# yitian97/SDformerFlow

Measured on AMD Instinct MI355X. Metric: event-frames/sec fwd (1x10x2x288x384), higher is better.
Workload: dtype f16x2; 1 GPU; BASELINE configs[1]: MS_SpikingformerFlowNet_en4 forward, batch 1 per GPU, 10-bin 288x384 voxel, neuron=lif; a step = one forward of one sample; 2 HIP streams per GPU, each replaying the HIP graph of one launch sequence that carries 10 independent batch-1 forwards of different voxels (replicas: every flow map bit-equal to a separate batch-1 forward, asserted by --full runs); one process per GPU; in_flight=2, replicas_per_launch=10, samples_in_flight=20, hip_graph=True, weight_planes=2

## Files before the change

sdformerflow_amd/csrc/ms_smallm.hip:

```cpp
#include "wide_common.h"
#include "switches.h"
#include <stdlib.h>

#ifdef SDF_STAMP
__device__ unsigned long long g_smallm_stamp[4 * 8];
__device__ unsigned long long g_smallm_census[2 * 1024];
#define MSTAMP(i) do { st[i] = __builtin_readcyclecounter(); } while (0)
#else
#define MSTAMP(i)
#endif

namespace sdfmm {
namespace {

struct SmallMParams {
  const uint8_t* A;
  const int8_t* W;
  const float* cscale;
  int N, K, HW;
  int64_t P;
  const float *bias, *alpha, *beta;
  const float* resid;
  float* out;
  int ldo;
  uint8_t* out_spike;
  int ldsp;
  SdfNeuronCfg sn;
  float inv_tau;
  int ncg, nunits;
  int cv_H, cv_W, cv_Cin, cv_spt;
  int cv_inv;
};

template <int T, int EPI, int NK, int AM, bool BT, int CB>
__global__ __launch_bounds__(256, CB == 2 ? 2 : 1) void smallm_kernel(SmallMParams P) {
  constexpr int RB = RBW, NS = CB == 2 ? 1 : 2, NBUF = NS + 1, ROWS = 16 * RB, SLOTS = 4 * RB, PPG = SLOTS / T, PPW = 4 * PPG, BN = 16 * CB;
  constexpr int SP1 = s_pitch(16), REDC = 3 * 2 * RB * 64 * 16;
  constexpr int STRIPB = 4 * RB * 1024, REDB = CB * REDC;
  static_assert(SLOTS % T == 0, "T must divide the 20 accumulator slots of a lane");
  static_assert(ROWS * SP1 <= REDC && STRIPB <= REDB, "the byte tiles and the strips lie inside the reduction buffer");
  __shared__ __attribute__((aligned(16))) uint8_t smem[REDB];
  __shared__ int32_t rowtab[ROWS];
  __shared__ uint32_t masktab[AM == 1 ? ROWS : 1];
  __shared__ __attribute__((aligned(16))) float psn_tbl[NK == 1 ? PSN_TABLE(T) : 4];
  const int tid = threadIdx.x, lane = tid & 63, wave = __builtin_amdgcn_readfirstlane(tid >> 6);
  const int l16 = lane & 15, lq = lane >> 4;
  int item = blockIdx.x;
  const int G = gridDim.x;
  if ((G & 7) == 0) item = (item & 7) * (G >> 3) + (item >> 3);
  if (item >= P.ncg * P.nunits) return;
#ifdef SDF_STAMP
  unsigned long long st[8] = {0, 0, 0, 0, 0, 0, 0, 0};
  const unsigned long long rt0 = __builtin_amdgcn_s_memrealtime();
  auto stamp_out = [&]() __attribute__((always_inline)) {
    asm volatile("s_waitcnt vmcnt(0)" ::: "memory");
    MSTAMP(5);
    if (lane == 0 && wave == 0 && blockIdx.x < 1024) {
      g_smallm_census[2 * blockIdx.x] = rt0;
      g_smallm_census[2 * blockIdx.x + 1] = __builtin_amdgcn_s_memrealtime();
    }
    if (lane == 0 && blockIdx.x == gridDim.x / 2) {
      unsigned long long* o = g_smallm_stamp + 8 * wave;
      for (int i = 0; i < 5; ++i) o[i] = st[i + 1] > st[i] ? st[i + 1] - st[i] : 0;
      o[5] = st[5] - st[0]; o[6] = __builtin_amdgcn_s_memrealtime() - rt0; o[7] = gridDim.x;
    }
  };
#endif
  MSTAMP(0);
  const int cg = item / P.nunits, unit = item - cg * P.nunits;
  const int n0 = cg * BN, K = P.K, N = P.N, HW = P.HW;
  const __amdgpu_buffer_rsrc_t A_rs = make_rsrc(P.A), W_rs = make_rsrc(P.W);
  const int nst = K >> 6;

  uint32_t pf[6] = {0, 0, 0, 0, 0, 0};
  if constexpr (BT) {
    const int per = G >> 3, first = (blockIdx.x & 7) * per;
    const uint32_t nw = 4u * (uint32_t)per, wi = 4u * (uint32_t)((blockIdx.x >> 3)) + (uint32_t)wave;
    const int cg_lo = first / P.nunits, cg_hi = min(P.ncg - 1, (first + per - 1) / P.nunits);
    const uint32_t cgb = (uint32_t)(CB * nst) * 3072u, wbase = (uint32_t)cg_lo * cgb, wlines = ((uint32_t)(cg_hi - cg_lo + 1) * cgb) >> 7;
    const uint32_t Lw = (wlines + nw - 1) / nw;
#pragma unroll
    for (int j = 0; j < 4; ++j) {
      const uint32_t ln = 64u * j + lane, line = wi * Lw + ln;
      pf[j] = __builtin_amdgcn_raw_buffer_load_b32(W_rs, (ln < Lw && line < wlines) ? wbase + line * 128u : INV, 0, 0);
    }
    const uint32_t alines = (uint32_t)(((int64_t)P.P * T * (AM == 1 ? P.cv_Cin : K)) >> 7), La = (alines + nw - 1) / nw;
#pragma unroll
    for (int j = 0; j < 2; ++j) {
      const uint32_t ln = 64u * j + lane, line = wi * La + ln;
      pf[4 + j] = __builtin_amdgcn_raw_buffer_load_b32(A_rs, (ln < La && line < alines) ? line * 128u : INV, 0, 0);
    }
  }

  if (tid < ROWS) {
    const int rb = tid >> 4, i = tid & 15, qq = i >> 2, slot = 4 * rb + (i & 3);
    const int pp = slot / T, t = slot - pp * T;
    const uint32_t pos = (uint32_t)unit * PPW + qq * PPG + pp;
    int32_t g = -1;
    if (pos < (uint32_t)P.P) {
      const uint32_t b = pos / (uint32_t)HW, hw = pos - b * (uint32_t)HW;
      g = (int32_t)((b * T + t) * (uint32_t)HW + hw);
    }
    rowtab[tid] = g;
    if constexpr (AM == 1) {
      uint32_t m = 0;
      if (g >= 0) {
        const uint32_t pix = (uint32_t)g % (uint32_t)HW, y = pix / (uint32_t)P.cv_W, xx = pix - y * (uint32_t)P.cv_W;
#pragma unroll
        for (int tp = 0; tp < 9; ++tp) {
          const int yy = (int)y + tp / 3 - 1, xw = (int)xx + tp % 3 - 1;
          if (yy >= 0 && yy < P.cv_H && xw >= 0 && xw < P.cv_W) m |= 1u << tp;
        }
      }
      masktab[tid] = m;
    }
  }
  if constexpr (NK == 1) psn_stage<T>(psn_tbl, P.sn, tid, 256);
  __syncthreads();
  uint32_t a_base[RB], a_mask[RB], b_off[CB];
  const int lr = lane >> 2, lp = (lane & 3) ^ ((lr >> 2) & 2);
#pragma unroll
  for (int rb = 0; rb < RB; ++rb) {
    const int32_t g = rowtab[16 * rb + lr];
    a_base[rb] = INV;
    a_mask[rb] = 0;
    if (g >= 0) {
      if constexpr (AM == 1) {
        a_base[rb] = (uint32_t)g * (uint32_t)P.cv_Cin + 16u * lp;
        a_mask[rb] = masktab[16 * rb + lr];
      } else {
        a_base[rb] = (uint32_t)g * (uint32_t)K + 16u * lp;
      }
    }
  }
#pragma unroll
  for (int cb = 0; cb < CB; ++cb) {
    if constexpr (BT) b_off[cb] = n0 + 16 * cb < N ? (uint32_t)(((n0 >> 4) + cb) * nst) * 3072u + 16u * lane : INV;
    else b_off[cb] = n0 + 16 * cb + l16 < N ? (uint32_t)(n0 + 16 * cb + l16) * (uint32_t)K + 16u * lq : INV;
  }
  uint8_t* mystrip = smem + wave * (RB * 1024);
  const uint32_t rd_off = (uint32_t)((4 * l16 + (lq ^ ((l16 >> 2) & 2))) * 16), wr_off = 16u * lane;

  i32x4 acc[3][RB][CB];
#pragma unroll
  for (int dg = 0; dg < 3; ++dg)
#pragma unroll
    for (int rb = 0; rb < RB; ++rb)
#pragma unroll
      for (int cb = 0; cb < CB; ++cb) acc[dg][rb][cb] = i32x4{0, 0, 0, 0};

  constexpr bool DBL = CB == 3;
  i32x4 araw[NS][RB], a2[DBL ? 2 : 1][RB], b[NBUF][3][CB];
  int sa_next = wave, sb_next = wave;
  const uint32_t plane = (uint32_t)N * (uint32_t)K;
#ifdef SMX_NOA
  constexpr bool XA = false;
#else
  constexpr bool XA = true;
#endif
#ifdef SMX_NOB
  constexpr bool XB = false;
#else
  constexpr bool XB = true;
#endif
  auto issue_a1 = [&](int ra, int rb) __attribute__((always_inline)) {
    if constexpr (AM == 1) {
      const int tap = (int)(((uint32_t)sa_next * (uint32_t)P.cv_inv) >> 16), cstep = sa_next - tap * P.cv_spt;
      const uint32_t toff = (uint32_t)(((tap / 3 - 1) * P.cv_W + (tap % 3 - 1)) * P.cv_Cin), cin0 = (uint32_t)cstep * 64u;
      const uint32_t ok = (0u - ((a_mask[rb] >> tap) & 1u)) & (0u - (uint32_t)XA);
      araw[ra][rb] = __builtin_bit_cast(i32x4, __builtin_amdgcn_raw_buffer_load_b128(A_rs, ((a_base[rb] + toff) & ok) | (INV & ~ok), cin0, 0));
    } else {
      const bool in = XA && sa_next < nst;
      araw[ra][rb] = __builtin_bit_cast(i32x4, __builtin_amdgcn_raw_buffer_load_b128(A_rs, in ? a_base[rb] : INV, (uint32_t)sa_next * 64u, 0));
    }
  };
  auto issue_b1 = [&](int rbuf, int f) __attribute__((always_inline)) {
    const bool in = XB && sb_next < nst;
    const int dg = f / CB, cb = f - dg * CB;
    const uint32_t so = BT ? (uint32_t)(sb_next * 3 + dg) * 1024u : (uint32_t)dg * plane + (uint32_t)sb_next * 64u;
    b[rbuf][dg][cb] = __builtin_bit_cast(i32x4, __builtin_amdgcn_raw_buffer_load_b128(W_rs, in ? b_off[cb] : INV, so, 0));
  };
  auto strip_write1 = [&](int ra, int rb) __attribute__((always_inline)) {
    *reinterpret_cast<i32x4*>(mystrip + rb * 1024 + wr_off) = araw[ra][rb];
  };
  auto strip_read1 = [&](int set, int rb) __attribute__((always_inline)) {
    a2[set][rb] = *reinterpret_cast<const i32x4*>(mystrip + rb * 1024 + rd_off);
  };
  auto step = [&](int i) __attribute__((always_inline)) {
    const int cur = DBL ? (i & 1) : 0, nxt = DBL ? (cur ^ 1) : 0;
#pragma unroll
    for (int g = 0; g < 3 * CB; ++g) {
      const int dg = g / CB, cb = g - dg * CB;
#pragma unroll
      for (int rb = 0; rb < RB; ++rb) {
#ifndef SMX_NOMFMA
        mfma_i8(acc[dg][rb][cb], a2[cur][rb], b[i % NBUF][dg][cb]);
#else
        asm volatile("" :: "v"(a2[cur][rb]), "v"(b[i % NBUF][dg][cb]));
#endif
        if (g == 0) strip_write1((i + 1) % NS, rb);
        if (g == 1) issue_a1((i + 1) % NS, rb);
        if (g == 2 && DBL) strip_read1(nxt, rb);
        if (g >= 1 && rb == (g == 1 ? RB - 1 : 0)) issue_b1(i % NBUF, g - 1);
        __builtin_amdgcn_sched_barrier(0);
      }
    }
    sa_next += 4;
    issue_b1(i % NBUF, 3 * CB - 1);
    sb_next += 4;
    if (!DBL) {
#pragma unroll
      for (int rb = 0; rb < RB; ++rb) strip_read1(nxt, rb);
    }
    __builtin_amdgcn_sched_barrier(0);
  };
  MSTAMP(1);
#pragma unroll
  for (int j = 0; j < NS; ++j) {
#pragma unroll
    for (int rb = 0; rb < RB; ++rb) issue_a1(j, rb);
    sa_next += 4;
  }
#pragma unroll
  for (int j = 0; j < NBUF; ++j) {
#pragma unroll
    for (int f = 0; f < 3 * CB; ++f) issue_b1(j, f);
    sb_next += 4;
  }
  asm volatile("" :: "v"(pf[0]), "v"(pf[1]), "v"(pf[2]), "v"(pf[3]), "v"(pf[4]), "v"(pf[5]));
#pragma unroll
  for (int rb = 0; rb < RB; ++rb) strip_write1(0, rb);
#pragma unroll
  for (int rb = 0; rb < RB; ++rb) issue_a1(0, rb);
  sa_next += 4;
#pragma unroll
  for (int rb = 0; rb < RB; ++rb) strip_read1(0, rb);
  __builtin_amdgcn_sched_barrier(0);
  constexpr int U = DBL ? 6 : 2;
  static_assert(U % NS == 0 && U % NBUF == 0, "ring sizes divide the round");
  const int nrounds = ((nst + 3) / 4 + U - 1) / U;
#pragma unroll 1
  for (int r = 0; r < nrounds; ++r) {
#pragma unroll
    for (int j = 0; j < U; ++j) step(j);
  }
  mfma_drain(acc);

  MSTAMP(2);
  const int c = lane & 15, q = lane >> 4;
  const bool owner = wave < CB;
  const int mycb = owner ? wave : 0;
  uint32_t xo[SLOTS];
  float res[SLOTS];
  float al = 1.f, be = 0.f, bs = 0.f, cs = 0.f;
  const int ncol = n0 + 16 * mycb + c;
  if (owner) {
#pragma unroll
    for (int s = 0; s < SLOTS; ++s) {
      const int32_t g = rowtab[16 * (s >> 2) + 4 * q + (s & 3)];
      xo[s] = (g >= 0 && ncol < N) ? ((uint32_t)g * (uint32_t)P.ldo + (uint32_t)ncol) * 4u : INV;
    }
    const __amdgpu_buffer_rsrc_t r_rs = make_rsrc(P.resid);
#pragma unroll
    for (int s = 0; s < SLOTS; ++s) res[s] = __builtin_bit_cast(float, __builtin_amdgcn_raw_buffer_load_b32(r_rs, P.resid ? xo[s] : INV, 0, 0));
    const int nc = ncol < N ? ncol : 0;
    al = P.alpha ? P.alpha[nc] : 1.f;
    be = P.alpha ? P.beta[nc] : 0.f;
    bs = P.bias ? P.bias[nc] : 0.f;
    cs = P.cscale[nc];
  }
  i32x4* red = reinterpret_cast<i32x4*>(smem);
  __builtin_amdgcn_sched_barrier(0);
  __syncthreads();
  __builtin_amdgcn_sched_barrier(0);
#pragma unroll
  for (int cb = 0; cb < CB; ++cb)
    if (wave != cb) {
      const int j = wave < cb ? wave : wave - 1;
#pragma unroll
      for (int rb = 0; rb < RB; ++rb) {
        red[(((cb * 3 + j) * 2 + 0) * RB + rb) * 64 + lane] = acc_read(acc[1][rb][cb]) * 256 + acc_read(acc[0][rb][cb]);
        red[(((cb * 3 + j) * 2 + 1) * RB + rb) * 64 + lane] = acc_read(acc[2][rb][cb]);
        __builtin_amdgcn_sched_barrier(0);
      }
    }
  __syncthreads();
  MSTAMP(3);
#ifdef SDF_STAMP
  if (!owner) { st[4] = st[3]; stamp_out(); return; }
#else
  if (!owner) return;
#endif
  const __amdgpu_buffer_rsrc_t x_rs = make_rsrc(P.out), o_rs = make_rsrc(P.out_spike);
  float val[SLOTS];
#pragma unroll
  for (int rb = 0; rb < RB; ++rb) {
    i32x4 lo = i32x4{0, 0, 0, 0}, hi = i32x4{0, 0, 0, 0};
#pragma unroll
    for (int cb = 0; cb < CB; ++cb)
      if (wave == cb) { lo = acc_read(acc[1][rb][cb]) * 256 + acc_read(acc[0][rb][cb]); hi = acc_read(acc[2][rb][cb]); }
#pragma unroll
    for (int j = 0; j < 3; ++j) {
      lo += red[(((mycb * 3 + j) * 2 + 0) * RB + rb) * 64 + lane];
      hi += red[(((mycb * 3 + j) * 2 + 1) * RB + rb) * 64 + lane];
    }
#pragma unroll
    for (int e = 0; e < 4; ++e) {
      const int s = 4 * rb + e;
      float v = __builtin_fmaf((float)hi[e], 65536.f, (float)lo[e]) * cs;
      v = v + bs;
      v = __builtin_fmaf(v, al, be);
      v = v + res[s];
      val[s] = v;
      if constexpr ((EPI & 2) != 0) __builtin_amdgcn_raw_buffer_store_b32(__builtin_bit_cast(uint32_t, v), x_rs, xo[s], 0, 0);
    }
    __builtin_amdgcn_sched_barrier(0);
  }
  if constexpr ((EPI & 1) != 0) {
    uint8_t* S = smem + mycb * REDC;
    uint32_t sel1, sel2;
    quad_sel(lane, sel1, sel2);
    const int m4 = (c >> 2), ci = c & 3;
    uint32_t bits = 0;
#pragma unroll
    for (int pp = 0; pp < PPG; ++pp) {
      float xs[T], sp[T];
#pragma unroll
      for (int t = 0; t < T; ++t) xs[t] = val[pp * T + t];
      neuron_any<NK, T>(xs, sp, P.sn, P.inv_tau, psn_tbl);
#pragma unroll
      for (int t = 0; t < T; ++t) bits |= ((__float_as_uint(sp[t]) >> 29) & 1u) << (pp * T + t);
    }
#pragma unroll
    for (int rb = 0; rb < RB; ++rb) {
      const uint32_t w = quad_tr_bytes(spread4(bits >> (4 * rb)), sel1, sel2);
      *reinterpret_cast<uint32_t*>(S + (16 * rb + 4 * q + ci) * SP1 + 4 * m4) = w;
    }
#pragma unroll
    for (int it = 0; it < (ROWS + 63) / 64; ++it) {
      const int r = lane + 64 * it;
      if (r < ROWS) {
        const int32_t g = rowtab[r];
        const u32x4 v = *reinterpret_cast<const u32x4*>(S + r * SP1);
        const uint32_t off = (g >= 0 && n0 + 16 * mycb < N) ? (uint32_t)g * (uint32_t)P.ldsp + (uint32_t)(n0 + 16 * mycb) : INV;
        __builtin_amdgcn_raw_buffer_store_b128(v, o_rs, off, 0, 0);
      }
    }
  }
#ifdef SDF_STAMP
  MSTAMP(4);
  stamp_out();
#endif
}

template <int T, int AM, bool BT, int CB>
void launch_t(const SmallMParams& P, int epi, int nk, dim3 grid, hipStream_t s) {
  if (epi == 2) SDF_LAUNCH((smallm_kernel<T, 2, 0, AM, BT, CB>), grid, dim3(256), 0, s, P);
  else if (epi == 1) {
    if (nk == 0) SDF_LAUNCH((smallm_kernel<T, 1, 0, AM, BT, CB>), grid, dim3(256), 0, s, P);
    else if (nk == 1) SDF_LAUNCH((smallm_kernel<T, 1, 1, AM, BT, CB>), grid, dim3(256), 0, s, P);
    else SDF_LAUNCH((smallm_kernel<T, 1, 2, AM, BT, CB>), grid, dim3(256), 0, s, P);
  } else {
    if (nk == 0) SDF_LAUNCH((smallm_kernel<T, 3, 0, AM, BT, CB>), grid, dim3(256), 0, s, P);
    else if (nk == 1) SDF_LAUNCH((smallm_kernel<T, 3, 1, AM, BT, CB>), grid, dim3(256), 0, s, P);
    else SDF_LAUNCH((smallm_kernel<T, 3, 2, AM, BT, CB>), grid, dim3(256), 0, s, P);
  }
}

template <int T, int AM>
void launch_bt(const SmallMParams& P, int epi, int nk, bool bt, int cb, dim3 grid, hipStream_t s) {
  if (bt) { if (cb == 3) launch_t<T, AM, true, 3>(P, epi, nk, grid, s); else launch_t<T, AM, true, 2>(P, epi, nk, grid, s); }
  else launch_t<T, AM, false, 2>(P, epi, nk, grid, s);
}

__global__ __launch_bounds__(256) void tile_weight_i8x3_kernel(const int8_t* __restrict__ planes, int8_t* __restrict__ tiled, int N, int K) {
  const int64_t i = (int64_t)blockIdx.x * 256 + threadIdx.x, total = (int64_t)3 * N * (K >> 4);
  if (i >= total) return;
  const int lane = (int)(i & 63);
  int64_t f = i >> 6;
  const int p = (int)(f % 3);
  f /= 3;
  const int nst = K >> 6, st = (int)(f % nst), cbk = (int)(f / nst);
  const int8_t* src = planes + ((int64_t)p * N + 16 * cbk + (lane & 15)) * K + 64 * st + 16 * (lane >> 4);
  *reinterpret_cast<u32x4*>(tiled + i * 16) = *reinterpret_cast<const u32x4*>(src);
}

}

static bool smallm_neuron_ok(const SdfNeuronCfg& n) {
  if (n.kind == SDF_PSN) return n.psn_w != nullptr && n.psn_b != nullptr;
  if (n.kind != SDF_LIF && n.kind != SDF_IF) return false;
  return sdf_tau_ok(n.kind, n.tau);
}

constexpr int64_t SMALLM_MAX_ROWS = 64 * 80;
static int64_t smallm_conv_rows() {
  if (const char* e = sdf_sw(SW_SMALLM_CONV_ROWS)) { const long v = atol(e); if (v >= 80) return v; }
  return 400 * 80;
}

bool smallm_conv_supports(const GemmParams& P) {
  const SdfSpikeGemmDesc& d = P.d;
  const ConvGeom& cv = P.cv;
  if (const char* e = sdf_sw(SW_SMALLM)) { if (e[0] == '0') return false; }
  if ((d.nsplit != SDF_PLANES_I8X3 && d.nsplit != SDF_PLANES_I8X3_TILED) || !d.col_scale) return false;
  if (cv.KWc != 3 || d.K != 9 * cv.Cin || cv.Cin % 64 || cv.sy != 1 || cv.sx != 1 || cv.OH != cv.H || cv.OW != cv.W) return false;
  if (cv.dy[0] != -1 || cv.dy[1] != 0 || cv.dy[2] != 1 || cv.dx[0] != -1 || cv.dx[1] != 0 || cv.dx[2] != 1) return false;
  if (d.N % 32 || d.out_rowmap || d.bias || d.add || d.zg_nH) return false;
  const int64_t hw = (int64_t)cv.H * cv.W, imgs = d.M / hw;
  int T = d.sn_T;
  if (T == 0) T = imgs % 10 == 0 ? 10 : (imgs % 20 == 0 ? 20 : 0);
  if (T != 10 && T != 20) return false;
  if (imgs % T || d.M > smallm_conv_rows()) return false;
  if (d.sn_T > 0) {
    if (!smallm_neuron_ok({d.sn_kind, d.tau, d.v_th, d.v_reset, d.soft_reset, d.psn_w, d.psn_b})) return false;
    if (d.pos_inner != hw || d.t_stride != hw || d.pos_ostride != (int64_t)T * hw || d.pos_count * T != d.M) return false;
    if (!d.out_spike) return false;
  } else if (!d.out) {
    return false;
  }
  if (d.M * (int64_t)cv.Cin >= (1LL << 31) || d.M * (int64_t)d.N * 4 >= (1LL << 31) || (int64_t)d.N * d.K * 3 >= (1LL << 31)) return false;
  return sdf_aligned(d.A, 16) && sdf_aligned(d.Wp, 16) && (!d.out || sdf_aligned(d.out, 16)) && (!d.resid || sdf_aligned(d.resid, 16)) &&
         (!d.out_spike || sdf_aligned(d.out_spike, 16)) && (!d.out || d.ldo == d.N);
}

int launch_smallm_conv(const GemmParams& G, hipStream_t s) {
  const SdfSpikeGemmDesc& d = G.d;
  const ConvGeom& cv = G.cv;
  const int64_t hw = (int64_t)cv.H * cv.W, imgs = d.M / hw;
  int T = d.sn_T;
  if (T == 0) T = imgs % 10 == 0 ? 10 : 20;
  SmallMParams P = {};
  P.A = d.A; P.W = reinterpret_cast<const int8_t*>(d.Wp); P.cscale = d.col_scale; P.N = d.N; P.K = d.K; P.HW = (int)hw; P.P = (imgs / T) * hw;
  P.alpha = d.alpha; P.beta = d.beta; P.resid = d.resid; P.out = d.out; P.ldo = d.N;
  P.out_spike = d.sn_T > 0 ? d.out_spike : nullptr; P.ldsp = d.N;
  P.sn = {d.sn_kind, d.tau, d.v_th, d.v_reset, d.soft_reset, d.psn_w, d.psn_b};
  P.inv_tau = d.sn_T > 0 ? inv_tau_of(P.sn) : 0.f;
  P.cv_H = cv.H; P.cv_W = cv.W; P.cv_Cin = cv.Cin; P.cv_spt = cv.Cin / 64;
  P.cv_inv = (65536 + P.cv_spt - 1) / P.cv_spt;
  for (int st = 0; st < 9 * P.cv_spt + 64; ++st)
    if ((int)(((uint32_t)st * (uint32_t)P.cv_inv) >> 16) != st / P.cv_spt) return SDF_E_SHAPE;
  const int PPW = 4 * (20 / T);
  P.nunits = (int)((P.P + PPW - 1) / PPW);
  const bool bt = d.nsplit == SDF_PLANES_I8X3_TILED;
  int cb = 2;
  if (const char* e = sdf_sw(SW_SMALLM_CB)) { if (bt && e[0] == '3' && d.N % 48 == 0) cb = 3; else if (e[0] == '2') cb = 2; }
  P.ncg = d.N / (16 * cb);
  const int64_t items = (int64_t)P.ncg * P.nunits;
  const dim3 grid((unsigned)((items + 7) / 8 * 8));
  const int epi = d.sn_T > 0 ? (d.out ? 3 : 1) : 2, nk = d.sn_T > 0 ? neuron_class(P.sn) : 0;
  if (T == 10) launch_bt<10, 1>(P, epi, nk, bt, cb, grid, s); else launch_bt<20, 1>(P, epi, nk, bt, cb, grid, s);
  hipError_t e = hipGetLastError();
  return e != hipSuccess ? (int)e : 0;
}

bool smallm_fc2_supports(const SdfMsMlpDesc* d) {
  if (const char* e = sdf_sw(SW_SMALLM)) { if (e[0] == '0') return false; }
  if (const char* e = sdf_sw(SW_SMALLM_FC2)) { if (e[0] == '0') return false; }
  if (!d->fc2_tiled || !d->fc2_cscale || (d->D != 10 && d->D != 20) || d->Ch % 64 || d->C % 32) return false;
  const int64_t tokens = (int64_t)d->B * d->D * d->HW;
  if (tokens > SMALLM_MAX_ROWS || tokens * d->Ch >= (1LL << 31) || tokens * d->C * 4 >= (1LL << 31) || (int64_t)d->C * d->Ch * 3 >= (1LL << 31)) return false;
  if (d->emit_next && !smallm_neuron_ok(d->emit_sn)) return false;
  {
    const int64_t ppw = 4 * (20 / d->D), units = ((int64_t)d->B * d->HW + ppw - 1) / ppw;
    const char* e = sdf_sw(SW_SMALLM_FC2);
    if (units * (d->C / 32) > 512 && !(e && e[0] == '2')) return false;
  }
  return sdf_aligned(d->fc2_tiled, 16) && sdf_aligned(d->x, 16) && (!d->emit_next || sdf_aligned(d->emit_next, 16));
}

int launch_smallm_fc2(const SdfMsMlpDesc* d, const uint8_t* s2, hipStream_t s) {
  SmallMParams P = {};
  P.A = s2; P.W = d->fc2_tiled; P.cscale = d->fc2_cscale; P.N = d->C; P.K = d->Ch; P.HW = (int)d->HW; P.P = (int64_t)d->B * d->HW;
  P.alpha = d->fc2_alpha; P.beta = d->fc2_beta; P.resid = d->x; P.out = d->x; P.ldo = d->C;
  P.out_spike = d->emit_next; P.ldsp = d->C; P.sn = d->emit_sn; P.inv_tau = d->emit_next ? inv_tau_of(d->emit_sn) : 0.f;
  const int T = d->D, PPW = 4 * (20 / T);
  P.nunits = (int)((P.P + PPW - 1) / PPW);
  P.ncg = d->C / 32;
  const int64_t items = (int64_t)P.ncg * P.nunits;
  if (items >= (1LL << 31) - 8) return SDF_E_SHAPE;
  const dim3 grid((unsigned)((items + 7) / 8 * 8));
  const int epi = d->emit_next ? 3 : 2, nk = d->emit_next ? neuron_class(d->emit_sn) : 0;
  if (T == 10) launch_t<10, 0, true, 2>(P, epi, nk, grid, s); else launch_t<20, 0, true, 2>(P, epi, nk, grid, s);
  hipError_t e = hipGetLastError();
  return e != hipSuccess ? (int)e : 0;
}

bool smallm_gemm_supports(const GemmParams& P) {
  const SdfSpikeGemmDesc& d = P.d;
  if (const char* e = sdf_sw(SW_SMALLM)) { if (e[0] == '0') return false; }
  if (d.nsplit != SDF_PLANES_I8X3_TILED || !d.col_scale || d.sn_T > 0 || !d.out) return false;
  if (d.K % 64 || d.K < 64 || d.N % 32 || d.lda != d.K || d.out_rowmap || d.add || d.zg_nH) return false;
  if (d.M % 10 || d.M > smallm_conv_rows()) return false;
  if (d.M * (int64_t)d.K >= (1LL << 31) || d.M * (int64_t)d.ldo * 4 >= (1LL << 31) || (int64_t)d.N * d.K * 3 >= (1LL << 31)) return false;
  return sdf_aligned(d.A, 16) && sdf_aligned(d.Wp, 16) && sdf_aligned(d.out, 16) && (!d.resid || sdf_aligned(d.resid, 16)) && d.ldo >= d.N;
}

int launch_smallm_gemm(const GemmParams& G, hipStream_t s) {
  const SdfSpikeGemmDesc& d = G.d;
  SmallMParams P = {};
  P.A = d.A; P.W = reinterpret_cast<const int8_t*>(d.Wp); P.cscale = d.col_scale; P.N = d.N; P.K = d.K; P.HW = (int)(d.M / 10); P.P = d.M / 10;
  P.alpha = d.alpha; P.beta = d.beta; P.bias = d.bias; P.resid = d.resid; P.out = d.out; P.ldo = (int)d.ldo;
  P.nunits = (int)((P.P + 7) / 8);
  int cb = 2;
  if (const char* e = sdf_sw(SW_SMALLM_CB)) { if (e[0] == '3' && d.N % 48 == 0) cb = 3; else if (e[0] == '2') cb = 2; }
  P.ncg = d.N / (16 * cb);
  const int64_t items = (int64_t)P.ncg * P.nunits;
  if (items >= (1LL << 31) - 8) return SDF_E_SHAPE;
  const dim3 grid((unsigned)((items + 7) / 8 * 8));
  if (cb == 3) SDF_LAUNCH((smallm_kernel<10, 2, 0, 0, true, 3>), grid, dim3(256), 0, s, P);
  else SDF_LAUNCH((smallm_kernel<10, 2, 0, 0, true, 2>), grid, dim3(256), 0, s, P);
  hipError_t e = hipGetLastError();
  return e != hipSuccess ? (int)e : 0;
}

}

#ifdef SDF_STAMP
extern "C" int sdf_debug_read_stamps_smallm(unsigned long long* host32, unsigned long long* census) {
  (void)hipMemcpyFromSymbol(census, HIP_SYMBOL(g_smallm_census), sizeof(g_smallm_census));
  return (int)hipMemcpyFromSymbol(host32, HIP_SYMBOL(g_smallm_stamp), sizeof(g_smallm_stamp));
}
#endif

extern "C" int sdf_tile_weight_i8x3(const int8_t* planes, int8_t* tiled, int N, int K, void* stream) {
  if (!planes || !tiled) return SDF_E_NULL;
  if (N < 16 || N % 16 || K < 64 || K % 64 || (int64_t)3 * N * K >= (1LL << 31)) return SDF_E_SHAPE;
  if (!sdf_aligned(planes, 16) || !sdf_aligned(tiled, 16)) return SDF_E_ALIGN;
  const int64_t total = (int64_t)3 * N * (K >> 4);
  SDF_LAUNCH(sdfmm::tile_weight_i8x3_kernel, dim3((unsigned)((total + 255) / 256)), dim3(256), 0, sdf_stream(stream), planes, tiled, N, K);
  SDF_LAUNCH_CHECK();
  return 0;
}
```

sdformerflow_amd/csrc/switches.h:

```cpp
#pragma once
#define SDF_SWITCH_LIST(X)                                                                                                        \
  X(DENSE_TPW) X(DENSE_LINEAR_XCD) X(HEAD_MFMA) X(MLP_FUSED_ANY) X(MLP_FUSED) X(RES) X(RES_STRIP) X(RES_UPW) X(RES_RMUL)            \
  X(RES_MINC) X(RES_MAXC) X(SMALLM) X(SMALLM_CONV_ROWS) X(SMALLM_CB) X(SMALLM_FC2) X(WIDE) X(WIDE_CB) X(WIDE_PASSES)                \
  X(WIDE_MAXROWS) X(WIDE_CONV) X(QK_FRONT) X(QK_FRONT_ANY) X(CONV_WRES) X(CONV_WRES_RB) X(CONV_WRES_GROUPS) X(CONV_WRES_CB_INNER)   \
  X(CONV_WRES_NOSPK) X(CONV_MULTI) X(DECONV_WRES) X(DECONV_BALANCE) X(DECONV_EPI) X(GEMM_CFG) X(GEMM_WGS) X(PP_PAIR)     \
  X(ATTN_GENERIC) X(ATTN_F32) X(KSPLIT_MULT) X(GEMM_WS)
enum SdfSwitch {
#define X(n) SW_##n,
  SDF_SWITCH_LIST(X)
#undef X
      SW_COUNT
};
const char* sdf_sw(SdfSwitch s);
```

Before: 831.7 samples/s.

## Process two row units per block in small-M spike GEMM to reuse weight loads

After: 808.1 samples/s. -2.8%, worse.

```diff
diff --git a/sdformerflow_amd/csrc/ms_smallm.hip b/sdformerflow_amd/csrc/ms_smallm.hip
--- a/sdformerflow_amd/csrc/ms_smallm.hip
+++ b/sdformerflow_amd/csrc/ms_smallm.hip
@@ -32,13 +32,15 @@
   int cv_inv;
 };
 
-template <int T, int EPI, int NK, int AM, bool BT, int CB>
-__global__ __launch_bounds__(256, CB == 2 ? 2 : 1) void smallm_kernel(SmallMParams P) {
-  constexpr int RB = RBW, NS = CB == 2 ? 1 : 2, NBUF = NS + 1, ROWS = 16 * RB, SLOTS = 4 * RB, PPG = SLOTS / T, PPW = 4 * PPG, BN = 16 * CB;
+template <int T, int EPI, int NK, int AM, bool BT, int CB, int UR = 1>
+__global__ __launch_bounds__(256, CB == 2 && UR == 1 ? 2 : 1) void smallm_kernel(SmallMParams P) {
+  constexpr int RB = RBW, RBT = UR * RB, NS = CB == 2 ? 1 : 2, NBUF = NS + 1, ROWS = 16 * RBT, ROWSU = 16 * RB, SLOTS = 4 * RB, PPG = SLOTS / T,
+                PPW = 4 * PPG, BN = 16 * CB, NOWN = UR * CB;
   constexpr int SP1 = s_pitch(16), REDC = 3 * 2 * RB * 64 * 16;
-  constexpr int STRIPB = 4 * RB * 1024, REDB = CB * REDC;
+  constexpr int STRIPB = 4 * RBT * 1024, REDB = NOWN * REDC;
   static_assert(SLOTS % T == 0, "T must divide the 20 accumulator slots of a lane");
-  static_assert(ROWS * SP1 <= REDC && STRIPB <= REDB, "the byte tiles and the strips lie inside the reduction buffer");
+  static_assert(NOWN <= 4 && ROWS <= 256, "one wave finishes each (unit, column block) output; one thread per tile row");
+  static_assert(ROWSU * SP1 <= REDC && STRIPB <= REDB, "the byte tiles and the strips lie inside the reduction buffer");
   __shared__ __attribute__((aligned(16))) uint8_t smem[REDB];
   __shared__ int32_t rowtab[ROWS];
   __shared__ uint32_t masktab[AM == 1 ? ROWS : 1];
@@ -93,9 +95,9 @@
   }
 
   if (tid < ROWS) {
-    const int rb = tid >> 4, i = tid & 15, qq = i >> 2, slot = 4 * rb + (i & 3);
+    const int rb = tid >> 4, i = tid & 15, qq = i >> 2, u = rb / RB, slot = 4 * (rb - u * RB) + (i & 3);
     const int pp = slot / T, t = slot - pp * T;
-    const uint32_t pos = (uint32_t)unit * PPW + qq * PPG + pp;
+    const uint32_t pos = ((uint32_t)unit * UR + u) * PPW + qq * PPG + pp;
     int32_t g = -1;
     if (pos < (uint32_t)P.P) {
       const uint32_t b = pos / (uint32_t)HW, hw = pos - b * (uint32_t)HW;
@@ -117,10 +119,10 @@
   }
   if constexpr (NK == 1) psn_stage<T>(psn_tbl, P.sn, tid, 256);
   __syncthreads();
-  uint32_t a_base[RB], a_mask[RB], b_off[CB];
+  uint32_t a_base[RBT], a_mask[RBT], b_off[CB];
   const int lr = lane >> 2, lp = (lane & 3) ^ ((lr >> 2) & 2);
 #pragma unroll
-  for (int rb = 0; rb < RB; ++rb) {
+  for (int rb = 0; rb < RBT; ++rb) {
     const int32_t g = rowtab[16 * rb + lr];
     a_base[rb] = INV;
     a_mask[rb] = 0;
@@ -138,19 +140,19 @@
     if constexpr (BT) b_off[cb] = n0 + 16 * cb < N ? (uint32_t)(((n0 >> 4) + cb) * nst) * 3072u + 16u * lane : INV;
     else b_off[cb] = n0 + 16 * cb + l16 < N ? (uint32_t)(n0 + 16 * cb + l16) * (uint32_t)K + 16u * lq : INV;
   }
-  uint8_t* mystrip = smem + wave * (RB * 1024);
+  uint8_t* mystrip = smem + wave * (RBT * 1024);
   const uint32_t rd_off = (uint32_t)((4 * l16 + (lq ^ ((l16 >> 2) & 2))) * 16), wr_off = 16u * lane;
 
-  i32x4 acc[3][RB][CB];
+  i32x4 acc[3][RBT][CB];
 #pragma unroll
   for (int dg = 0; dg < 3; ++dg)
 #pragma unroll
-    for (int rb = 0; rb < RB; ++rb)
+    for (int rb = 0; rb < RBT; ++rb)
 #pragma unroll
       for (int cb = 0; cb < CB; ++cb) acc[dg][rb][cb] = i32x4{0, 0, 0, 0};
 
-  constexpr bool DBL = CB == 3;
-  i32x4 araw[NS][RB], a2[DBL ? 2 : 1][RB], b[NBUF][3][CB];
+  constexpr bool DBL = CB == 3 || UR > 1;
+  i32x4 araw[NS][RBT], a2[DBL ? 2 : 1][RBT], b[NBUF][3][CB];
   int sa_next = wave, sb_next = wave;
   const uint32_t plane = (uint32_t)N * (uint32_t)K;
 #ifdef SMX_NOA
@@ -192,7 +194,7 @@
     for (int g = 0; g < 3 * CB; ++g) {
       const int dg = g / CB, cb = g - dg * CB;
 #pragma unroll
-      for (int rb = 0; rb < RB; ++rb) {
+      for (int rb = 0; rb < RBT; ++rb) {
 #ifndef SMX_NOMFMA
         mfma_i8(acc[dg][rb][cb], a2[cur][rb], b[i % NBUF][dg][cb]);
 #else
@@ -201,7 +203,7 @@
         if (g == 0) strip_write1((i + 1) % NS, rb);
         if (g == 1) issue_a1((i + 1) % NS, rb);
         if (g == 2 && DBL) strip_read1(nxt, rb);
-        if (g >= 1 && rb == (g == 1 ? RB - 1 : 0)) issue_b1(i % NBUF, g - 1);
+        if (g >= 1 && rb == (g == 1 ? RBT - 1 : 0)) issue_b1(i % NBUF, g - 1);
         __builtin_amdgcn_sched_barrier(0);
       }
     }
@@ -210,7 +212,7 @@
     sb_next += 4;
     if (!DBL) {
 #pragma unroll
-      for (int rb = 0; rb < RB; ++rb) strip_read1(nxt, rb);
+      for (int rb = 0; rb < RBT; ++rb) strip_read1(nxt, rb);
     }
     __builtin_amdgcn_sched_barrier(0);
   };
@@ -218,7 +220,7 @@
 #pragma unroll
   for (int j = 0; j < NS; ++j) {
 #pragma unroll
-    for (int rb = 0; rb < RB; ++rb) issue_a1(j, rb);
+    for (int rb = 0; rb < RBT; ++rb) issue_a1(j, rb);
     sa_next += 4;
   }
 #pragma unroll
@@ -229,27 +231,27 @@
   }
   asm volatile("" :: "v"(pf[0]), "v"(pf[1]), "v"(pf[2]), "v"(pf[3]), "v"(pf[4]), "v"(pf[5]));
 #pragma unroll
-  for (int rb = 0; rb < RB; ++rb) strip_write1(0, rb);
-#pragma unroll
-  for (int rb = 0; rb < RB; ++rb) issue_a1(0, rb);
+  for (int rb = 0; rb < RBT; ++rb) strip_write1(0, rb);
+#pragma unroll
+  for (int rb = 0; rb < RBT; ++rb) issue_a1(0, rb);
   sa_next += 4;
 #pragma unroll
-  for (int rb = 0; rb < RB; ++rb) strip_read1(0, rb);
+  for (int rb = 0; rb < RBT; ++rb) strip_read1(0, rb);
   __builtin_amdgcn_sched_barrier(0);
-  constexpr int U = DBL ? 6 : 2;
-  static_assert(U % NS == 0 && U % NBUF == 0, "ring sizes divide the round");
-  const int nrounds = ((nst + 3) / 4 + U - 1) / U;
+  constexpr int RND = CB == 3 ? 6 : 2;
+  static_assert(RND % NS == 0 && RND % NBUF == 0 && RND % 2 == 0, "ring sizes divide the round");
+  const int nrounds = ((nst + 3) / 4 + RND - 1) / RND;
 #pragma unroll 1
   for (int r = 0; r < nrounds; ++r) {
 #pragma unroll
-    for (int j = 0; j < U; ++j) step(j);
+    for (int j = 0; j < RND; ++j) step(j);
   }
   mfma_drain(acc);
 
   MSTAMP(2);
   const int c = lane & 15, q = lane >> 4;
-  const bool owner = wave < CB;
-  const int mycb = owner ? wave : 0;
+  const bool owner = wave < NOWN;
+  const int myob = owner ? wave : 0, myu = myob / CB, mycb = myob - myu * CB;
   uint32_t xo[SLOTS];
   float res[SLOTS];
   float al = 1.f, be = 0.f, bs = 0.f, cs = 0.f;
@@ -257,7 +259,7 @@
   if (owner) {
 #pragma unroll
     for (int s = 0; s < SLOTS; ++s) {
-      const int32_t g = rowtab[16 * (s >> 2) + 4 * q + (s & 3)];
+      const int32_t g = rowtab[ROWSU * myu + 16 * (s >> 2) + 4 * q + (s & 3)];
       xo[s] = (g >= 0 && ncol < N) ? ((uint32_t)g * (uint32_t)P.ldo + (uint32_t)ncol) * 4u : INV;
     }
     const __amdgpu_buffer_rsrc_t r_rs = make_rsrc(P.resid);
@@ -274,13 +276,13 @@
   __syncthreads();
   __builtin_amdgcn_sched_barrier(0);
 #pragma unroll
-  for (int cb = 0; cb < CB; ++cb)
-    if (wave != cb) {
-      const int j = wave < cb ? wave : wave - 1;
+  for (int ob = 0; ob < NOWN; ++ob)
+    if (wave != ob) {
+      const int j = wave < ob ? wave : wave - 1, r0 = (ob / CB) * RB, cb = ob % CB;
 #pragma unroll
       for (int rb = 0; rb < RB; ++rb) {
-        red[(((cb * 3 + j) * 2 + 0) * RB + rb) * 64 + lane] = acc_read(acc[1][rb][cb]) * 256 + acc_read(acc[0][rb][cb]);
-        red[(((cb * 3 + j) * 2 + 1) * RB + rb) * 64 + lane] = acc_read(acc[2][rb][cb]);
+        red[(((ob * 3 + j) * 2 + 0) * RB + rb) * 64 + lane] = acc_read(acc[1][r0 + rb][cb]) * 256 + acc_read(acc[0][r0 + rb][cb]);
+        red[(((ob * 3 + j) * 2 + 1) * RB + rb) * 64 + lane] = acc_read(acc[2][r0 + rb][cb]);
         __builtin_amdgcn_sched_barrier(0);
       }
     }
@@ -297,12 +299,16 @@
   for (int rb = 0; rb < RB; ++rb) {
     i32x4 lo = i32x4{0, 0, 0, 0}, hi = i32x4{0, 0, 0, 0};
 #pragma unroll
-    for (int cb = 0; cb < CB; ++cb)
-      if (wave == cb) { lo = acc_read(acc[1][rb][cb]) * 256 + acc_read(acc[0][rb][cb]); hi = acc_read(acc[2][rb][cb]); }
+    for (int ob = 0; ob < NOWN; ++ob)
+      if (wave == ob) {
+        const int r = (ob / CB) * RB + rb, cb = ob % CB;
+        lo = acc_read(acc[1][r][cb]) * 256 + acc_read(acc[0][r][cb]);
+        hi = acc_read(acc[2][r][cb]);
+      }
 #pragma unroll
     for (int j = 0; j < 3; ++j) {
-      lo += red[(((mycb * 3 + j) * 2 + 0) * RB + rb) * 64 + lane];
-      hi += red[(((mycb * 3 + j) * 2 + 1) * RB + rb) * 64 + lane];
+      lo += red[(((myob * 3 + j) * 2 + 0) * RB + rb) * 64 + lane];
+      hi += red[(((myob * 3 + j) * 2 + 1) * RB + rb) * 64 + lane];
     }
 #pragma unroll
     for (int e = 0; e < 4; ++e) {
@@ -317,7 +323,7 @@
     __builtin_amdgcn_sched_barrier(0);
   }
   if constexpr ((EPI & 1) != 0) {
-    uint8_t* S = smem + mycb * REDC;
+    uint8_t* S = smem + myob * REDC;
     uint32_t sel1, sel2;
     quad_sel(lane, sel1, sel2);
     const int m4 = (c >> 2), ci = c & 3;
@@ -337,10 +343,10 @@
       *reinterpret_cast<uint32_t*>(S + (16 * rb + 4 * q + ci) * SP1 + 4 * m4) = w;
     }
 #pragma unroll
-    for (int it = 0; it < (ROWS + 63) / 64; ++it) {
+    for (int it = 0; it < (ROWSU + 63) / 64; ++it) {
       const int r = lane + 64 * it;
-      if (r < ROWS) {
-        const int32_t g = rowtab[r];
+      if (r < ROWSU) {
+        const int32_t g = rowtab[ROWSU * myu + r];
         const u32x4 v = *reinterpret_cast<const u32x4*>(S + r * SP1);
         const uint32_t off = (g >= 0 && n0 + 16 * mycb < N) ? (uint32_t)g * (uint32_t)P.ldsp + (uint32_t)(n0 + 16 * mycb) : INV;
         __builtin_amdgcn_raw_buffer_store_b128(v, o_rs, off, 0, 0);
@@ -371,6 +377,26 @@
 void launch_bt(const SmallMParams& P, int epi, int nk, bool bt, int cb, dim3 grid, hipStream_t s) {
   if (bt) { if (cb == 3) launch_t<T, AM, true, 3>(P, epi, nk, grid, s); else launch_t<T, AM, true, 2>(P, epi, nk, grid, s); }
   else launch_t<T, AM, false, 2>(P, epi, nk, grid, s);
+}
+
+template <int T, int AM>
+void launch_rows(const SmallMParams& P, int epi, int nk, dim3 grid, hipStream_t s) {
+  if (epi == 2) SDF_LAUNCH((smallm_kernel<T, 2, 0, AM, true, 2, 2>), grid, dim3(256), 0, s, P);
+  else if (epi == 1) {
+    if (nk == 0) SDF_LAUNCH((smallm_kernel<T, 1, 0, AM, true, 2, 2>), grid, dim3(256), 0, s, P);
+    else SDF_LAUNCH((smallm_kernel<T, 1, 2, AM, true, 2, 2>), grid, dim3(256), 0, s, P);
+  } else {
+    if (nk == 0) SDF_LAUNCH((smallm_kernel<T, 3, 0, AM, true, 2, 2>), grid, dim3(256), 0, s, P);
+    else SDF_LAUNCH((smallm_kernel<T, 3, 2, AM, true, 2, 2>), grid, dim3(256), 0, s, P);
+  }
+}
+
+constexpr int SMALLM_UR = 2;
+static bool smallm_many_rows(int64_t units, int ncg, int K) {
+  const char* e = sdf_sw(SW_SMALLM_ROWS);
+  if (K < 64 || K % 64 || units < SMALLM_UR || (e && e[0] == '0')) return false;
+  if (e && e[0] == '2') return true;
+  return (units + SMALLM_UR - 1) / SMALLM_UR * ncg >= 2 * 256;
 }
 
 __global__ __launch_bounds__(256) void tile_weight_i8x3_kernel(const int8_t* __restrict__ planes, int8_t* __restrict__ tiled, int N, int K) {
@@ -446,10 +472,13 @@
   int cb = 2;
   if (const char* e = sdf_sw(SW_SMALLM_CB)) { if (bt && e[0] == '3' && d.N % 48 == 0) cb = 3; else if (e[0] == '2') cb = 2; }
   P.ncg = d.N / (16 * cb);
+  const int epi = d.sn_T > 0 ? (d.out ? 3 : 1) : 2, nk = d.sn_T > 0 ? neuron_class(P.sn) : 0;
+  const bool rows = bt && cb == 2 && nk != 1 && smallm_many_rows(P.nunits, P.ncg, d.K);
+  if (rows) P.nunits = (P.nunits + SMALLM_UR - 1) / SMALLM_UR;
   const int64_t items = (int64_t)P.ncg * P.nunits;
   const dim3 grid((unsigned)((items + 7) / 8 * 8));
-  const int epi = d.sn_T > 0 ? (d.out ? 3 : 1) : 2, nk = d.sn_T > 0 ? neuron_class(P.sn) : 0;
-  if (T == 10) launch_bt<10, 1>(P, epi, nk, bt, cb, grid, s); else launch_bt<20, 1>(P, epi, nk, bt, cb, grid, s);
+  if (rows) { if (T == 10) launch_rows<10, 1>(P, epi, nk, grid, s); else launch_rows<20, 1>(P, epi, nk, grid, s); }
+  else if (T == 10) launch_bt<10, 1>(P, epi, nk, bt, cb, grid, s); else launch_bt<20, 1>(P, epi, nk, bt, cb, grid, s);
   hipError_t e = hipGetLastError();
   return e != hipSuccess ? (int)e : 0;
 }
@@ -505,10 +534,13 @@
   int cb = 2;
   if (const char* e = sdf_sw(SW_SMALLM_CB)) { if (e[0] == '3' && d.N % 48 == 0) cb = 3; else if (e[0] == '2') cb = 2; }
   P.ncg = d.N / (16 * cb);
+  const bool rows = cb == 2 && smallm_many_rows(P.nunits, P.ncg, d.K);
+  if (rows) P.nunits = (P.nunits + SMALLM_UR - 1) / SMALLM_UR;
   const int64_t items = (int64_t)P.ncg * P.nunits;
   if (items >= (1LL << 31) - 8) return SDF_E_SHAPE;
   const dim3 grid((unsigned)((items + 7) / 8 * 8));
-  if (cb == 3) SDF_LAUNCH((smallm_kernel<10, 2, 0, 0, true, 3>), grid, dim3(256), 0, s, P);
+  if (rows) SDF_LAUNCH((smallm_kernel<10, 2, 0, 0, true, 2, 2>), grid, dim3(256), 0, s, P);
+  else if (cb == 3) SDF_LAUNCH((smallm_kernel<10, 2, 0, 0, true, 3>), grid, dim3(256), 0, s, P);
   else SDF_LAUNCH((smallm_kernel<10, 2, 0, 0, true, 2>), grid, dim3(256), 0, s, P);
   hipError_t e = hipGetLastError();
   return e != hipSuccess ? (int)e : 0;
diff --git a/sdformerflow_amd/csrc/switches.h b/sdformerflow_amd/csrc/switches.h
--- a/sdformerflow_amd/csrc/switches.h
+++ b/sdformerflow_amd/csrc/switches.h
@@ -1,7 +1,7 @@
 #pragma once
 #define SDF_SWITCH_LIST(X)                                                                                                        \
   X(DENSE_TPW) X(DENSE_LINEAR_XCD) X(HEAD_MFMA) X(MLP_FUSED_ANY) X(MLP_FUSED) X(RES) X(RES_STRIP) X(RES_UPW) X(RES_RMUL)            \
-  X(RES_MINC) X(RES_MAXC) X(SMALLM) X(SMALLM_CONV_ROWS) X(SMALLM_CB) X(SMALLM_FC2) X(WIDE) X(WIDE_CB) X(WIDE_PASSES)                \
+  X(RES_MINC) X(RES_MAXC) X(SMALLM) X(SMALLM_CONV_ROWS) X(SMALLM_CB) X(SMALLM_ROWS) X(SMALLM_FC2) X(WIDE) X(WIDE_CB) X(WIDE_PASSES)                \
   X(WIDE_MAXROWS) X(WIDE_CONV) X(QK_FRONT) X(QK_FRONT_ANY) X(CONV_WRES) X(CONV_WRES_RB) X(CONV_WRES_GROUPS) X(CONV_WRES_CB_INNER)   \
   X(CONV_WRES_NOSPK) X(CONV_MULTI) X(DECONV_WRES) X(DECONV_BALANCE) X(DECONV_EPI) X(GEMM_CFG) X(GEMM_WGS) X(PP_PAIR)     \
   X(ATTN_GENERIC) X(ATTN_F32) X(KSPLIT_MULT) X(GEMM_WS)
```
